# jcorsetti/oryon

Hardware: AMD Instinct MI355X
Metric: image-pairs/sec end-to-end (feat+match+reg) @224², C=256; ADD(-S) parity (higher is better)
Workload: dtype f32

## Files before the change

### oryon_amd/csrc/screen_mx6.hip

```cpp
#include <hip/hip_runtime.h>
#include <stdio.h>
#include <stdlib.h>
#include <type_traits>
#include "common.h"
#include "match_common.h"
#include "screen_tile.h"

namespace oryon {

typedef int i32x8 __attribute__((ext_vector_type(8)));
typedef float f32x16s __attribute__((ext_vector_type(16)));

template <int CP, int WAVES = 8, int VAR = 0>
__global__ __launch_bounds__(64 * WAVES, CP == 512 ? 1 : 2) void match_mx6_screen_kernel(
    const uint8_t *__restrict__ a6, const uint8_t *__restrict__ q6, int B, int cap_a, int cap_q, const int32_t *__restrict__ n_a,
    const int32_t *__restrict__ n_q, int T, int S, float *__restrict__ ws_max, int32_t *__restrict__ ws_i1, float *__restrict__ ws_m2)
{
    constexpr int RB = CP;
    constexpr int TILE_BYTES = screen8_tile_bytes(CP);
    constexpr int NQB = 4, NAB = 2;
    constexpr int NKS = CP / 64;
    constexpr int NI = TILE_BYTES / (1024 * WAVES);
    char *smem;
    if constexpr (2 * TILE_BYTES > 65536) {
        extern __shared__ __attribute__((aligned(256))) char smem_dyn6[];
        smem = smem_dyn6;
    } else {
        __shared__ __attribute__((aligned(256))) char smem_st6[2 * TILE_BYTES];
        smem = smem_st6;
    }
    ScreenUnit u;
    if (!screen_unit_decode(u, 64 * WAVES, B, T, S, n_a, n_q)) return;
    const int p = u.p, split = u.split, a0 = u.a0;
    int qt_begin, qt_end;
    screen_split_tiles(u, S, qt_begin, qt_end);
    const int t = threadIdx.x, lane = t & 63, wave = t >> 6, l31 = lane & 31, hi = lane >> 5;
    const char *qp = reinterpret_cast<const char *>(q6) + (size_t)p * cap_q * RB;

    i32x8 breg[NAB][NKS];
#pragma unroll
    for (int ab = 0; ab < NAB; ++ab) {
        const int arow_i = a0 + wave * 64 + ab * 32 + l31;
        const char *arow = reinterpret_cast<const char *>(a6) + ((size_t)p * cap_a + (arow_i < cap_a ? arow_i : cap_a - 1)) * RB + 32 * hi;
#pragma unroll
        for (int s = 0; s < NKS; ++s) {
            const i32x4 lo = *reinterpret_cast<const i32x4 *>(arow + 64 * s), up = *reinterpret_cast<const i32x4 *>(arow + 64 * s + 16);
            breg[ab][s] = __builtin_shufflevector(lo, up, 0, 1, 2, 3, 4, 5, 6, 7);
        }
    }
    unsigned dma_off[NI];
    screen_dma_offsets<RB>(dma_off, wave * NI, lane);
    const int wave_u = __builtin_amdgcn_readfirstlane(wave);
    auto issue_one = [&](int qt, int buf, int j) {
        const char *qb = qp + (size_t)qt * TILE_BYTES;
        char *dst = smem + buf * TILE_BYTES + (wave_u * NI + j) * 1024;
        __builtin_amdgcn_global_load_lds((const __attribute__((address_space(1))) void *)(qb + dma_off[j]),
                                         (__attribute__((address_space(3))) void *)dst, 16, 0, 0);
    };
    unsigned koff[4][2];
#pragma unroll
    for (int c = 0; c < 4; ++c)
#pragma unroll
        for (int e = 0; e < 2; ++e) koff[c][e] = (unsigned)(l31 * RB) + ((((unsigned)(4 * c + 2 * hi + e)) ^ (unsigned)(l31 & 15)) << 4);
    auto rd = [&](int s, int qb, unsigned tile) -> i32x8 {
        const unsigned base = tile + (unsigned)(qb * 32 * RB + (s >> 2) * 256);
        const i32x4 lo = *reinterpret_cast<const i32x4 *>(smem + koff[s & 3][0] + base);
        const i32x4 up = *reinterpret_cast<const i32x4 *>(smem + koff[s & 3][1] + base);
        return __builtin_shufflevector(lo, up, 0, 1, 2, 3, 4, 5, 6, 7);
    };

    float runmax[NAB], run2[NAB];
    int runidx[NAB];
#pragma unroll
    for (int ab = 0; ab < NAB; ++ab) { runmax[ab] = -INFINITY; run2[ab] = -INFINITY; runidx[ab] = 0; }
    auto reduce_block = [&](const f32x16s &c, int sid, int ab) {
        if constexpr (VAR == 1) { runmax[ab] = fmaxf(runmax[ab], c[0] + c[15]); runidx[ab] = sid; return; }
        const float m0 = fmaxf(fmaxf(c[0], c[1]), c[2]), m1 = fmaxf(fmaxf(c[3], c[4]), c[5]), m2 = fmaxf(fmaxf(c[6], c[7]), c[8]);
        const float m3 = fmaxf(fmaxf(c[9], c[10]), c[11]), m4 = fmaxf(fmaxf(c[12], c[13]), c[14]);
        const float x = fmaxf(fmaxf(fmaxf(m0, m1), m2), fmaxf(fmaxf(m3, m4), c[15]));
        const bool improved = x > runmax[ab];
        run2[ab] = __builtin_amdgcn_fmed3f(runmax[ab], run2[ab], x);
        runmax[ab] = fmaxf(runmax[ab], x);
        runidx[ab] = improved ? sid : runidx[ab];
    };
    const f32x16s zero16 = {0, 0, 0, 0, 0, 0, 0, 0, 0, 0, 0, 0, 0, 0, 0, 0};

    if (qt_end > qt_begin) {
#pragma unroll
        for (int j = 0; j < NI; ++j) issue_one(qt_begin, 0, j);
    }
    asm volatile("s_waitcnt vmcnt(0)" ::: "memory");
    __syncthreads();

    i32x8 areg[NKS];
#pragma unroll
    for (int s = 0; s < NKS; ++s) areg[s] = rd(s, 0, 0u);
    f32x16s prev[NAB];
#pragma unroll
    for (int ab = 0; ab < NAB; ++ab)
#pragma unroll
        for (int r = 0; r < 16; ++r) prev[ab][r] = -3.0e38f;
    int prev_sid = 0;
    auto do_tile = [&](int qt, auto BUFC) {
        constexpr int BUF = decltype(BUFC)::value;
        constexpr unsigned tile = BUF * TILE_BYTES;
        const int qt_next = qt + 1 < qt_end ? qt + 1 : qt;
#pragma unroll
        for (int qb = 0; qb < NQB; ++qb) {
            f32x16s acc[NAB];
            if (qb == 0) {
#pragma unroll
                for (int j = 0; j < NI; ++j) issue_one(qt_next, BUF ^ 1, j);
            }
#pragma unroll
            for (int s = 0; s < NKS; ++s) {
#pragma unroll
                for (int ab = 0; ab < NAB; ++ab)
                    acc[ab] = __builtin_amdgcn_mfma_scale_f32_32x32x64_f8f6f4(areg[s], breg[ab][s], s == 0 ? zero16 : acc[ab], 2, 2, 0,
                                                                               areg[s][6], 0, breg[ab][s][6]);
                if (qb + 1 < NQB) areg[s] = rd(s, qb + 1, tile);
            }
#pragma unroll
            for (int ab = 0; ab < NAB; ++ab) reduce_block(prev[ab], prev_sid, ab);
#pragma unroll
            for (int i = 0; i < NKS; ++i) {
                __builtin_amdgcn_sched_group_barrier(0x008, 1, 0);
                __builtin_amdgcn_sched_group_barrier(0x002, 24 / (2 * NKS), 0);
                __builtin_amdgcn_sched_group_barrier(0x008, 1, 0);
                __builtin_amdgcn_sched_group_barrier(0x002, 24 / (2 * NKS), 0);
                if (qb + 1 < NQB) __builtin_amdgcn_sched_group_barrier(0x100, 2, 0);
            }
#pragma unroll
            for (int ab = 0; ab < NAB; ++ab) prev[ab] = acc[ab];
            prev_sid = (qt * NQB + qb) * 2 + hi;
        }
        asm volatile("s_waitcnt vmcnt(0)" ::: "memory");
        __syncthreads();
#pragma unroll
        for (int s = 0; s < NKS; ++s) areg[s] = rd(s, 0, (BUF ^ 1) * TILE_BYTES);
    };
    for (int qt = qt_begin; qt < qt_end; qt += 2) {
        do_tile(qt, std::integral_constant<int, 0>{});
        if (qt + 1 < qt_end) do_tile(qt + 1, std::integral_constant<int, 1>{});
    }
#pragma unroll
    for (int ab = 0; ab < NAB; ++ab) reduce_block(prev[ab], prev_sid, ab);
    screen_merge_store<NAB>(runmax, run2, runidx, a0 + wave * 64 + l31, hi, (size_t)p * S + split, cap_a, ws_max, ws_i1, ws_m2);
}


template <int S0, int N, class F>
__device__ __forceinline__ void mx6_static_for(F &&f)
{
    if constexpr (S0 < N) {
        f(std::integral_constant<int, S0>{});
        mx6_static_for<S0 + 1, N>(f);
    }
}

struct Mx6RowList {
    const int32_t *idx;
    int idx_stride, stride, cap_src;
    int n;
};
struct Mx6RowsInPlace {};

template <int CP, int WAVES, int KL, bool IDX = false>
__device__ __forceinline__ void mx6_screen_w4_tiles(char *smem, const uint8_t *__restrict__ a6, const uint8_t *__restrict__ q6, int p, int split,
                                                    int a0, int cap_a, int cap_q, int S, int qt_begin, int qt_end, float *__restrict__ ws_max,
                                                    int32_t *__restrict__ ws_i1, float *__restrict__ ws_m2,
                                                    const std::conditional_t<IDX, Mx6RowList, Mx6RowsInPlace> &rows = {})
{
    static_assert(CP == 256 || (CP == 512 && WAVES == 4), "geometries: C_pad 256 with 4 / 8 waves, C_pad 512 with 4 waves");
    constexpr int RB = CP, NAB = 4;
    constexpr int TILE_BYTES = screen8_tile_bytes(CP);
    constexpr int NQB = 4;
    constexpr int NKS = CP / 64;
    constexpr int NI = TILE_BYTES / (1024 * WAVES);
    constexpr int LPR = RB / 256;
    const int t = threadIdx.x, lane = t & 63, wave = t >> 6, l31 = lane & 31, hi = lane >> 5;
    const char *qp = reinterpret_cast<const char *>(q6) + (size_t)p * cap_q * RB;

    i32x8 breg[NAB][NKS];
    int bsc[NAB][NKS / 4];
#pragma unroll
    for (int ab = 0; ab < NAB; ++ab) {
        const int arow_i = a0 + wave * (32 * NAB) + ab * 32 + l31;
        const char *arow;
        bool live = true;
        if constexpr (IDX) {
            live = arow_i < rows.n;
            const int src = !live ? 0 : rows.idx ? rows.idx[(size_t)p * rows.idx_stride + arow_i] : arow_i * rows.stride;
            arow = reinterpret_cast<const char *>(a6) + ((size_t)p * rows.cap_src + src) * RB + 32 * hi;
        } else
            arow = reinterpret_cast<const char *>(a6) + ((size_t)p * cap_a + (arow_i < cap_a ? arow_i : cap_a - 1)) * RB + 32 * hi;
        unsigned sc[NKS / 4];
#pragma unroll
        for (int w = 0; w < NKS / 4; ++w) sc[w] = 0;
#pragma unroll
        for (int s = 0; s < KL; ++s) {
            i32x4 lo = *reinterpret_cast<const i32x4 *>(arow + 64 * s), up = *reinterpret_cast<const i32x4 *>(arow + 64 * s + 16);
            if constexpr (IDX) {
                const i32x4 z = {0, 0, 0, 0};
                lo = live ? lo : z;
                up = live ? up : z;
            }
            breg[ab][s] = __builtin_shufflevector(lo, up, 0, 1, 2, 3, 4, 5, -1, -1);
            sc[s >> 2] |= ((unsigned)up[2] & 0xffu) << (8 * (s & 3));
        }
#pragma unroll
        for (int w = 0; w < NKS / 4; ++w) bsc[ab][w] = (int)sc[w];
    }
    constexpr int DJ = 4 * LPR;
    static_assert(NI % DJ == 0 || NI == DJ, "DMA instructions per wave and tile");
    unsigned dma_off[DJ];
    screen_dma_offsets<RB>(dma_off, wave * NI, lane);
    const int wave_u = __builtin_amdgcn_readfirstlane(wave);
    auto issue_one = [&](int qt, int buf, int j) {
        const char *qb = qp + (size_t)qt * TILE_BYTES + (j / DJ) * (16 * RB);
        char *dst = smem + buf * TILE_BYTES + (wave_u * NI + j) * 1024;
        __builtin_amdgcn_global_load_lds((const __attribute__((address_space(1))) void *)(qb + dma_off[j % DJ]),
                                         (__attribute__((address_space(3))) void *)dst, 16, 0, 0);
    };
    unsigned koff[4][2];
#pragma unroll
    for (int c = 0; c < 4; ++c)
#pragma unroll
        for (int e = 0; e < 2; ++e) koff[c][e] = (unsigned)(l31 * RB) + ((((unsigned)(4 * c + 2 * hi + e)) ^ (unsigned)(l31 & 15)) << 4);
    auto rd = [&](int s, int qb, unsigned tile) -> i32x8 {
        const unsigned base = tile + (unsigned)(qb * 32 * RB + (s >> 2) * 256);
        const i32x4 lo = *reinterpret_cast<const i32x4 *>(smem + koff[s & 3][0] + base);
        const i32x4 up = *reinterpret_cast<const i32x4 *>(smem + koff[s & 3][1] + base);
        return __builtin_shufflevector(lo, up, 0, 1, 2, 3, 4, 5, 6, -1);
    };

    float runmax[NAB], run2[NAB];
    int runidx[NAB];
#pragma unroll
    for (int ab = 0; ab < NAB; ++ab) { runmax[ab] = -INFINITY; run2[ab] = -INFINITY; runidx[ab] = 0; }
    auto reduce_block = [&](const f32x16s &c, int sid, int ab) {
        const float m0 = fmaxf(fmaxf(c[0], c[1]), c[2]), m1 = fmaxf(fmaxf(c[3], c[4]), c[5]), m2 = fmaxf(fmaxf(c[6], c[7]), c[8]);
        const float m3 = fmaxf(fmaxf(c[9], c[10]), c[11]), m4 = fmaxf(fmaxf(c[12], c[13]), c[14]);
        const float x = fmaxf(fmaxf(fmaxf(m0, m1), m2), fmaxf(fmaxf(m3, m4), c[15]));
        const bool improved = x > runmax[ab];
        run2[ab] = __builtin_amdgcn_fmed3f(runmax[ab], run2[ab], x);
        runmax[ab] = __builtin_amdgcn_fmed3f(runmax[ab], x, INFINITY);
        runidx[ab] = improved ? sid : runidx[ab];
    };
    const f32x16s zero16 = {0, 0, 0, 0, 0, 0, 0, 0, 0, 0, 0, 0, 0, 0, 0, 0};

    if (qt_end > qt_begin) {
#pragma unroll
        for (int j = 0; j < NI; ++j) issue_one(qt_begin, 0, j);
    }
    asm volatile("s_waitcnt vmcnt(0)" ::: "memory");
    __syncthreads();

    i32x8 areg[NKS];
#pragma unroll
    for (int s = 0; s < KL; ++s) areg[s] = rd(s, 0, 0u);
    f32x16s acc[NAB];
#pragma unroll
    for (int ab = 0; ab < NAB; ++ab)
#pragma unroll
        for (int r = 0; r < 16; ++r) acc[ab][r] = -3.0e38f;
    int sid23 = 0;

    auto mfma = [&](f32x16s &d, int ab, auto SC) {
        constexpr int s_ = decltype(SC)::value;
        d = __builtin_amdgcn_mfma_scale_f32_32x32x64_f8f6f4(areg[s_], breg[ab][s_], s_ == 0 ? zero16 : d, 2, 2, 0, areg[s_][6], s_ & 3,
                                                            bsc[ab][s_ >> 2]);
    };
    int buf = 0;
    for (int qt = qt_begin; qt < qt_end; ++qt) {
        const unsigned tile = buf * TILE_BYTES;
        const int qt_next = qt + 1 < qt_end ? qt + 1 : qt;
#pragma unroll
        for (int qb = 0; qb < NQB; ++qb) {
            const int sid = (qt * NQB + qb) * 2 + hi;
            if (qb == 0) {
#pragma unroll
                for (int j = 0; j < NI; ++j) issue_one(qt_next, buf ^ 1, j);
            }
            reduce_block(acc[2], sid23, 2);
            reduce_block(acc[3], sid23, 3);
            mx6_static_for<0, KL>([&](auto SC) { mfma(acc[0], 0, SC); mfma(acc[1], 1, SC); });
#pragma unroll
            for (int i = 0; i < 2 * KL; ++i) {
                __builtin_amdgcn_sched_group_barrier(0x008, 1, 0);
                __builtin_amdgcn_sched_group_barrier(0x002, 16 / KL, 0);
            }
            mx6_static_for<0, KL>([&](auto SC) {
                constexpr int s_ = decltype(SC)::value;
                mfma(acc[2], 2, SC); mfma(acc[3], 3, SC);
                if (qb + 1 < NQB) areg[s_] = rd(s_, qb + 1, tile);
            });
            reduce_block(acc[0], sid, 0);
            reduce_block(acc[1], sid, 1);
#pragma unroll
            for (int i = 0; i < 2 * KL; ++i) {
                __builtin_amdgcn_sched_group_barrier(0x008, 1, 0);
                __builtin_amdgcn_sched_group_barrier(0x002, 16 / KL, 0);
                if (qb + 1 < NQB && (i & 1)) __builtin_amdgcn_sched_group_barrier(0x100, 2, 0);
            }
            sid23 = sid;
        }
        asm volatile("s_waitcnt vmcnt(0)" ::: "memory");
        __syncthreads();
        buf ^= 1;
#pragma unroll
        for (int s = 0; s < KL; ++s) areg[s] = rd(s, 0, buf * TILE_BYTES);
    }
    reduce_block(acc[2], sid23, 2);
    reduce_block(acc[3], sid23, 3);
    screen_merge_store<NAB>(runmax, run2, runidx, a0 + wave * (32 * NAB) + l31, hi, (size_t)p * S + split, cap_a, ws_max, ws_i1, ws_m2);
}

template <int CP, int WAVES, int KL = CP / 64>
__global__ __launch_bounds__(64 * WAVES, CP == 512 ? 1 : 2) void match_mx6_screen_w4_kernel(
    const uint8_t *__restrict__ a6, const uint8_t *__restrict__ q6, int B, int cap_a, int cap_q, const int32_t *__restrict__ n_a,
    const int32_t *__restrict__ n_q, int T, int S, float *__restrict__ ws_max, int32_t *__restrict__ ws_i1, float *__restrict__ ws_m2,
    long long *__restrict__ dbg_wg )
{
    constexpr int TILE_BYTES = screen8_tile_bytes(CP);
    char *smem;
    if constexpr (2 * TILE_BYTES > 65536) {
        extern __shared__ __attribute__((aligned(256))) char smem_dyn_w4[];
        smem = smem_dyn_w4;
    } else {
        __shared__ __attribute__((aligned(256))) char smem_st_w4[2 * TILE_BYTES];
        smem = smem_st_w4;
    }
    ScreenUnit u;
    if (!screen_unit_decode(u, 128 * WAVES, B, T, S, n_a, n_q)) return;
    int qt_begin, qt_end;
    screen_split_tiles(u, S, qt_begin, qt_end);
    const long long tk0 = dbg_wg ? wall_clock64() : 0;
    mx6_screen_w4_tiles<CP, WAVES, KL>(smem, a6, q6, u.p, u.split, u.a0, cap_a, cap_q, S, qt_begin, qt_end, ws_max, ws_i1, ws_m2);
    if (dbg_wg && threadIdx.x == 0) {
        dbg_wg[(size_t)blockIdx.x * 4 + 0] = tk0;
        dbg_wg[(size_t)blockIdx.x * 4 + 1] = wall_clock64();
        dbg_wg[(size_t)blockIdx.x * 4 + 2] = (long long)__builtin_amdgcn_s_getreg((31 << 11) | 4);
        dbg_wg[(size_t)blockIdx.x * 4 + 3] = (long long)__builtin_amdgcn_s_getreg((31 << 11) | 20);
    }
}

template <int KL>
__global__ __launch_bounds__(256, 2) void match_mx6_screen_w4_list_kernel(
    const uint8_t *__restrict__ a6, const uint8_t *__restrict__ q6, int B, int cap_src, int cap_list, int cap_q, const int32_t *__restrict__ count,
    const int32_t *__restrict__ idx, int idx_stride, int stride, const int32_t *__restrict__ n_q, int T, int S, float *__restrict__ ws_max,
    int32_t *__restrict__ ws_i1, float *__restrict__ ws_m2)
{
    __shared__ __attribute__((aligned(256))) char smem_st_w4l[2 * screen8_tile_bytes(256)];
    ScreenUnit u;
    if (!screen_unit_decode(u, 512, B, T, S, count, n_q)) return;
    Mx6RowList rows = {idx, idx_stride, stride, cap_src, 0};
    const int listed = idx ? u.na : (u.na + stride - 1) / stride;
    rows.n = listed < cap_list ? listed : cap_list;
    if (u.a0 >= rows.n) return;
    int qt_begin, qt_end;
    screen_split_tiles(u, S, qt_begin, qt_end);
    mx6_screen_w4_tiles<256, 4, KL, true>(smem_st_w4l, a6, q6, u.p, u.split, u.a0, cap_list, cap_q, S, qt_begin, qt_end, ws_max, ws_i1, ws_m2, rows);
}

template <int CP, int WAVES, int KL = CP / 64>
__global__ __launch_bounds__(64 * WAVES, CP == 512 ? 1 : 2) void match_mx6_screen_w4_win_kernel(
    const uint8_t *__restrict__ a6, const uint8_t *__restrict__ q6, int B, int cap_a, int cap_q, const int32_t *__restrict__ n_a,
    const int32_t *__restrict__ n_q, int T, int S, float *__restrict__ ws_max, int32_t *__restrict__ ws_i1, float *__restrict__ ws_m2,
    const int32_t *__restrict__ gate , int win ,
    const int32_t *__restrict__ band ,
    int band_T )
{
    constexpr int TILE_BYTES = screen8_tile_bytes(CP);
    char *smem;
    if constexpr (2 * TILE_BYTES > 65536) {
        extern __shared__ __attribute__((aligned(256))) char smem_dyn_w4w[];
        smem = smem_dyn_w4w;
    } else {
        __shared__ __attribute__((aligned(256))) char smem_st_w4w[2 * TILE_BYTES];
        smem = smem_st_w4w;
    }
    ScreenUnit u;
    if (!screen_unit_decode(u, 128 * WAVES, B, T, S, n_a, n_q)) return;
    if (gate && gate[u.p * T + u.panel] == 0) return;
    int qt_begin, qt_end;
    screen_split_tiles(u, S, qt_begin, qt_end);
    if (win > 0 && qt_end - qt_begin > win) {
        const int cnt = qt_end - qt_begin, panels = (u.na + 128 * WAVES - 1) / (128 * WAVES);
        int k0 = (int)(((long long)(2 * u.panel + 1) * cnt) / (2 * panels)) - win / 2;
        k0 = k0 < 0 ? 0 : (k0 > cnt - win ? cnt - win : k0);
        qt_begin += k0;
        qt_end = qt_begin + win;
    }
    if (band) {
        const int first = band[(u.p * band_T + u.panel) * 2], cnt = band[(u.p * band_T + u.panel) * 2 + 1];
        const int per = (cnt + S - 1) / S;
        qt_begin = first + u.split * per;
        qt_end = (qt_begin + per < first + cnt) ? qt_begin + per : first + cnt;
    }
    mx6_screen_w4_tiles<CP, WAVES, KL>(smem, a6, q6, u.p, u.split, u.a0, cap_a, cap_q, S, qt_begin, qt_end, ws_max, ws_i1, ws_m2);
}

static int mx6_var()
{
    static const int var = dev_env_int("ORYON_MX6_VAR", 0);
    return var;
}

namespace {
int mx6_live_ksteps(int C_true) { return (C_true > 0 && C_true <= 64) ? 1 : (C_true > 0 && C_true <= 128) ? 2 : 4; }
template <class F>
void mx6_with_kl(int kl, F &&f)
{
    if (kl == 1) f(std::integral_constant<int, 1>{});
    else if (kl == 2) f(std::integral_constant<int, 2>{});
    else f(std::integral_constant<int, 4>{});
}

template <int CP>
void launch_screen_mx6_t(int groups, int T, hipStream_t st, const uint8_t *a6, const uint8_t *q6, int B, int cap_a, int cap_q, const int32_t *n_a,
                       const int32_t *n_q, int S, float *ws_max, int32_t *ws_i1, float *ws_m2, int kl = 4, bool gate_or_win = false,
                       const int32_t *gate = nullptr, int win = 0)
{
    constexpr size_t dyn = 2 * screen8_tile_bytes(CP) > 65536 ? 2 * screen8_tile_bytes(CP) : 0;
    constexpr int W_ = CP == 512 ? 4 : 8;
    const int Tw = (cap_a + 64 * W_ - 1) / (64 * W_);
    const int var = mx6_var();
    if (var == 1) {
        if (dyn) allow_dynamic_lds(reinterpret_cast<const void *>(&match_mx6_screen_kernel<CP, W_, 1>), (int)dyn);
        hipLaunchKernelGGL((match_mx6_screen_kernel<CP, W_, 1>), dim3(groups / T * Tw), dim3(64 * W_), dyn, st, a6, q6, B, cap_a, cap_q, n_a, n_q, Tw,
                           S, ws_max, ws_i1, ws_m2);
        return;
    }
    if constexpr (CP == 256) {
        if (var == 0) {
            const int T8 = (cap_a + 1023) / 1024;
            const int g8 = groups / T * T8;
            if (gate_or_win) {
                mx6_with_kl(kl, [&](auto KLC) {
                    hipLaunchKernelGGL((match_mx6_screen_w4_win_kernel<CP, 8, decltype(KLC)::value>), dim3(g8), dim3(512), 0, st, a6, q6, B, cap_a,
                                       cap_q, n_a, n_q, T8, S, ws_max, ws_i1, ws_m2, gate, win, static_cast<const int32_t *>(nullptr), 0);
                });
                return;
            }
            mx6_with_kl(kl, [&](auto KLC) {
                hipLaunchKernelGGL((match_mx6_screen_w4_kernel<CP, 8, decltype(KLC)::value>), dim3(g8), dim3(512), 0, st, a6, q6, B, cap_a, cap_q,
                                   n_a, n_q, T8, S, ws_max, ws_i1, ws_m2, static_cast<long long *>(nullptr));
            });
            return;
        }
        if (var == 3) {
            hipLaunchKernelGGL((match_mx6_screen_w4_kernel<CP, 4>), dim3(groups / T * Tw), dim3(256), 0, st, a6, q6, B, cap_a, cap_q, n_a, n_q, Tw, S,
                               ws_max, ws_i1, ws_m2, nullptr);
            return;
        }
    }
    if constexpr (CP == 512) {
        if (var == 0) {
            allow_dynamic_lds(reinterpret_cast<const void *>(&match_mx6_screen_w4_kernel<CP, 4>), (int)dyn);
            hipLaunchKernelGGL((match_mx6_screen_w4_kernel<CP, 4>), dim3(groups / T * Tw), dim3(256), dyn, st, a6, q6, B, cap_a, cap_q, n_a, n_q, Tw,
                               S, ws_max, ws_i1, ws_m2, nullptr);
            return;
        }
    }
    if (dyn) allow_dynamic_lds(reinterpret_cast<const void *>(&match_mx6_screen_kernel<CP, W_>), (int)dyn);
    hipLaunchKernelGGL((match_mx6_screen_kernel<CP, W_>), dim3(groups / T * Tw), dim3(64 * W_), dyn, st, a6, q6, B, cap_a, cap_q, n_a, n_q, Tw, S,
                       ws_max, ws_i1, ws_m2);
}
}

const char *screen_mx6_name(int C)
{
    if (C != 256) return mx6_var() == 0 ? "match_mx6_screen_w4_kernel<512, 4>" : "match_mx6_screen_kernel<512, 4, 0>";
    return mx6_var() == 0 ? "match_mx6_screen_w4_kernel<256, 8>" : mx6_var() == 3 ? "match_mx6_screen_w4_kernel<256, 4>" : mx6_var() == 1 ? "match_mx6_screen_kernel<256, 8, 1>" : "match_mx6_screen_kernel<256, 8, 0>";
}

void launch_screen_mx6(int C, int groups, int T, hipStream_t st, const uint8_t *a6, const uint8_t *q6, int B, int cap_a, int cap_q,
                       const int32_t *n_a, const int32_t *n_q, int S, float *ws_max, int32_t *ws_i1, float *ws_m2, int C_true,
                       int cascade, const int32_t *gate, int win)
{
    if (C == 256)
        launch_screen_mx6_t<256>(groups, T, st, a6, q6, B, cap_a, cap_q, n_a, n_q, S, ws_max, ws_i1, ws_m2, mx6_live_ksteps(C_true), cascade != 0,
                                 gate, win);
    else launch_screen_mx6_t<512>(groups, T, st, a6, q6, B, cap_a, cap_q, n_a, n_q, S, ws_max, ws_i1, ws_m2);
}

void launch_screen_mx6_list512(hipStream_t st, const uint8_t *a6, const uint8_t *q6, int B, int cap_src, int cap_list, int cap_q,
                               const int32_t *count, const int32_t *idx, int idx_stride, int stride, const int32_t *n_q, int S, float *ws_max,
                               int32_t *ws_i1, float *ws_m2, int C_true)
{
    const int T = (cap_list + 511) / 512;
    const int groups = ((B * S + 7) / 8) * 8 * T;
    mx6_with_kl(mx6_live_ksteps(C_true), [&](auto KLC) {
        hipLaunchKernelGGL((match_mx6_screen_w4_list_kernel<decltype(KLC)::value>), dim3(groups), dim3(256), 0, st, a6, q6, B, cap_src, cap_list,
                           cap_q, count, idx, idx_stride, stride, n_q, T, S, ws_max, ws_i1, ws_m2);
    });
}

void launch_screen_mx6_band512(hipStream_t st, const uint8_t *a6, const uint8_t *q6, int B, int cap_a, int cap_q, const int32_t *n_a,
                               const int32_t *n_q, int S, float *ws_max, int32_t *ws_i1, float *ws_m2, int C_true, const int32_t *band, int band_T)
{
    const int T = (cap_a + 511) / 512;
    const int groups = ((B * S + 7) / 8) * 8 * T;
    mx6_with_kl(mx6_live_ksteps(C_true), [&](auto KLC) {
        hipLaunchKernelGGL((match_mx6_screen_w4_win_kernel<256, 4, decltype(KLC)::value>), dim3(groups), dim3(256), 0, st, a6, q6, B, cap_a, cap_q,
                           n_a, n_q, T, S, ws_max, ws_i1, ws_m2, static_cast<const int32_t *>(nullptr), 0, band, band_T);
    });
}

}
```

### oryon_amd/csrc/screen_tile.h

```cpp
#pragma once
#include <hip/hip_runtime.h>
#include <stdint.h>

namespace oryon {

typedef int i32x4 __attribute__((ext_vector_type(4)));

constexpr int SCREEN8_ROWS = 128;
constexpr int screen8_tile_bytes(int CP) { return CP * SCREEN8_ROWS; }

struct ScreenUnit {
    int p, split, panel, a0, na, nq;
};
__device__ __forceinline__ bool screen_unit_decode(ScreenUnit &u, int panel_rows, int B, int T, int S, const int32_t *__restrict__ n_a,
                                                   const int32_t *__restrict__ n_q)
{
    const int xcd = blockIdx.x & 7, slot = blockIdx.x >> 3;
    const int unit = (slot / T) * 8 + xcd;
    if (unit >= B * S) return false;
    u.panel = slot % T;
    u.p = unit / S;
    u.split = unit % S;
    u.na = n_a[u.p];
    u.nq = n_q[u.p];
    u.a0 = u.panel * panel_rows;
    return u.a0 < u.na;
}
__device__ __forceinline__ void screen_split_tiles(const ScreenUnit &u, int S, int &qt_begin, int &qt_end)
{
    const int nqt = (u.nq + SCREEN8_ROWS - 1) / SCREEN8_ROWS;
    const int qt_per = (nqt + S - 1) / S;
    qt_begin = u.split * qt_per;
    qt_end = (qt_begin + qt_per < nqt) ? qt_begin + qt_per : nqt;
}

template <int RB, int N>
__device__ __forceinline__ void screen_dma_offsets(unsigned (&off)[N], int first, int lane)
{
    constexpr int LPR = RB / 256;
    static_assert(LPR >= 1, "rows are whole 256-byte lines");
#pragma unroll
    for (int j = 0; j < N; ++j) {
        const int line = (first + j) * 4 + (lane >> 4), sl = lane & 15;
        const int row = line / LPR;
        off[j] = (unsigned)(row * RB + (((line % LPR) * 16 + (sl ^ (row & 15))) << 4));
    }
}

template <int NAB>
__device__ __forceinline__ void screen_merge_store(const float (&runmax)[NAB], const float (&run2)[NAB], const int (&runidx)[NAB], int a_lane,
                                                   int hi, size_t unit, int cap_a, float *__restrict__ ws_max, int32_t *__restrict__ ws_i1,
                                                   float *__restrict__ ws_m2)
{
#pragma unroll
    for (int ab = 0; ab < NAB; ++ab) {
        const float om1 = __shfl_xor(runmax[ab], 32), om2 = __shfl_xor(run2[ab], 32);
        const int oi1 = __shfl_xor(runidx[ab], 32);
        const float m1 = fmaxf(runmax[ab], om1);
        const float m2 = fmaxf(fminf(runmax[ab], om1), fmaxf(run2[ab], om2));
        const int i1 = (om1 > runmax[ab]) ? oi1 : runidx[ab];
        const int a = a_lane + ab * 32;
        if (hi == 0 && a < cap_a) {
            const size_t o = unit * cap_a + a;
            ws_max[o] = m1;
            ws_i1[o] = i1;
            ws_m2[o] = m2;
        }
    }
}

}
```

Baseline: 23710.

## Skip dead A-row blocks on partial list panels in mx6 screen kernel

For list-indexed screening panels, rows are re-laid out so each 128-row level spans all waves, and the kernel is instantiated with 2, 3 or 4 live A blocks based on how many rows remain in the panel. Tail panels then issue fewer MFMAs and reductions instead of computing on zero-padded rows. The sched_group_barrier interleave is generalized to uneven halves. This adds extra template instantiations, which cost code size, and gives tail panels a different instruction schedule.

```diff
diff --git a/oryon_amd/csrc/screen_mx6.hip b/oryon_amd/csrc/screen_mx6.hip
--- a/oryon_amd/csrc/screen_mx6.hip
+++ b/oryon_amd/csrc/screen_mx6.hip
@@ -165,7 +165,7 @@
 };
 struct Mx6RowsInPlace {};
 
-template <int CP, int WAVES, int KL, bool IDX = false>
+template <int CP, int WAVES, int KL, bool IDX = false, int NABL = 4>
 __device__ __forceinline__ void mx6_screen_w4_tiles(char *smem, const uint8_t *__restrict__ a6, const uint8_t *__restrict__ q6, int p, int split,
                                                     int a0, int cap_a, int cap_q, int S, int qt_begin, int qt_end, float *__restrict__ ws_max,
                                                     int32_t *__restrict__ ws_i1, float *__restrict__ ws_m2,
@@ -173,6 +173,9 @@
 {
     static_assert(CP == 256 || (CP == 512 && WAVES == 4), "geometries: C_pad 256 with 4 / 8 waves, C_pad 512 with 4 waves");
     constexpr int RB = CP, NAB = 4;
+    static_assert(NABL == NAB || (IDX && NABL >= 2 && NABL < NAB), "live levels: 2 .. 4, fewer than 4 on list panels only");
+    constexpr int HA = (NABL + 1) / 2, HB = NABL - HA;
+    static_assert((16 * HB) % (HA * KL) == 0 && (16 * HA) % (HB * KL) == 0, "epilogue instructions per MFMA (sched_group_barrier)");
     constexpr int TILE_BYTES = screen8_tile_bytes(CP);
     constexpr int NQB = 4;
     constexpr int NKS = CP / 64;
@@ -184,8 +187,8 @@
     i32x8 breg[NAB][NKS];
     int bsc[NAB][NKS / 4];
 #pragma unroll
-    for (int ab = 0; ab < NAB; ++ab) {
-        const int arow_i = a0 + wave * (32 * NAB) + ab * 32 + l31;
+    for (int ab = 0; ab < NABL; ++ab) {
+        const int arow_i = IDX ? a0 + (ab * WAVES + wave) * 32 + l31 : a0 + wave * (32 * NAB) + ab * 32 + l31;
         const char *arow;
         bool live = true;
         if constexpr (IDX) {
@@ -261,7 +264,7 @@
     for (int s = 0; s < KL; ++s) areg[s] = rd(s, 0, 0u);
     f32x16s acc[NAB];
 #pragma unroll
-    for (int ab = 0; ab < NAB; ++ab)
+    for (int ab = 0; ab < NABL; ++ab)
 #pragma unroll
         for (int r = 0; r < 16; ++r) acc[ab][r] = -3.0e38f;
     int sid23 = 0;
@@ -282,26 +285,30 @@
 #pragma unroll
                 for (int j = 0; j < NI; ++j) issue_one(qt_next, buf ^ 1, j);
             }
-            reduce_block(acc[2], sid23, 2);
-            reduce_block(acc[3], sid23, 3);
-            mx6_static_for<0, KL>([&](auto SC) { mfma(acc[0], 0, SC); mfma(acc[1], 1, SC); });
-#pragma unroll
-            for (int i = 0; i < 2 * KL; ++i) {
+            if constexpr (HB > 0) reduce_block(acc[HA], sid23, HA);
+            if constexpr (HB > 1) reduce_block(acc[HA + 1], sid23, HA + 1);
+            mx6_static_for<0, KL>([&](auto SC) {
+                mfma(acc[0], 0, SC);
+                if constexpr (HA > 1) mfma(acc[1], 1, SC);
+            });
+#pragma unroll
+            for (int i = 0; i < HA * KL; ++i) {
                 __builtin_amdgcn_sched_group_barrier(0x008, 1, 0);
-                __builtin_amdgcn_sched_group_barrier(0x002, 16 / KL, 0);
+                __builtin_amdgcn_sched_group_barrier(0x002, 16 * HB / (HA * KL), 0);
             }
             mx6_static_for<0, KL>([&](auto SC) {
                 constexpr int s_ = decltype(SC)::value;
-                mfma(acc[2], 2, SC); mfma(acc[3], 3, SC);
+                if constexpr (HB > 0) mfma(acc[HA], HA, SC);
+                if constexpr (HB > 1) mfma(acc[HA + 1], HA + 1, SC);
                 if (qb + 1 < NQB) areg[s_] = rd(s_, qb + 1, tile);
             });
             reduce_block(acc[0], sid, 0);
-            reduce_block(acc[1], sid, 1);
-#pragma unroll
-            for (int i = 0; i < 2 * KL; ++i) {
+            if constexpr (HA > 1) reduce_block(acc[1], sid, 1);
+#pragma unroll
+            for (int i = 0; i < HB * KL; ++i) {
                 __builtin_amdgcn_sched_group_barrier(0x008, 1, 0);
-                __builtin_amdgcn_sched_group_barrier(0x002, 16 / KL, 0);
-                if (qb + 1 < NQB && (i & 1)) __builtin_amdgcn_sched_group_barrier(0x100, 2, 0);
+                __builtin_amdgcn_sched_group_barrier(0x002, 16 * HA / (HB * KL), 0);
+                if (qb + 1 < NQB && i % HB == HB - 1) __builtin_amdgcn_sched_group_barrier(0x100, 2, 0);
             }
             sid23 = sid;
         }
@@ -311,9 +318,10 @@
 #pragma unroll
         for (int s = 0; s < KL; ++s) areg[s] = rd(s, 0, buf * TILE_BYTES);
     }
-    reduce_block(acc[2], sid23, 2);
-    reduce_block(acc[3], sid23, 3);
-    screen_merge_store<NAB>(runmax, run2, runidx, a0 + wave * (32 * NAB) + l31, hi, (size_t)p * S + split, cap_a, ws_max, ws_i1, ws_m2);
+    if constexpr (HB > 0) reduce_block(acc[HA], sid23, HA);
+    if constexpr (HB > 1) reduce_block(acc[HA + 1], sid23, HA + 1);
+    screen_merge_store<NAB, NABL>(runmax, run2, runidx, a0 + (IDX ? wave * 32 : wave * (32 * NAB)) + l31, hi, (size_t)p * S + split, cap_a, ws_max,
+                                  ws_i1, ws_m2, IDX ? 32 * WAVES : 32);
 }
 
 template <int CP, int WAVES, int KL = CP / 64>
@@ -360,7 +368,16 @@
     if (u.a0 >= rows.n) return;
     int qt_begin, qt_end;
     screen_split_tiles(u, S, qt_begin, qt_end);
-    mx6_screen_w4_tiles<256, 4, KL, true>(smem_st_w4l, a6, q6, u.p, u.split, u.a0, cap_list, cap_q, S, qt_begin, qt_end, ws_max, ws_i1, ws_m2, rows);
+    const int levels = (rows.n - u.a0 + 127) >> 7;
+    if (levels >= 4) {
+        mx6_screen_w4_tiles<256, 4, KL, true, 4>(smem_st_w4l, a6, q6, u.p, u.split, u.a0, cap_list, cap_q, S, qt_begin, qt_end, ws_max, ws_i1, ws_m2, rows);
+        return;
+    }
+    if (levels == 3) {
+        mx6_screen_w4_tiles<256, 4, KL, true, 3>(smem_st_w4l, a6, q6, u.p, u.split, u.a0, cap_list, cap_q, S, qt_begin, qt_end, ws_max, ws_i1, ws_m2, rows);
+        return;
+    }
+    mx6_screen_w4_tiles<256, 4, KL, true, 2>(smem_st_w4l, a6, q6, u.p, u.split, u.a0, cap_list, cap_q, S, qt_begin, qt_end, ws_max, ws_i1, ws_m2, rows);
 }
 
 template <int CP, int WAVES, int KL = CP / 64>
diff --git a/oryon_amd/csrc/screen_tile.h b/oryon_amd/csrc/screen_tile.h
--- a/oryon_amd/csrc/screen_tile.h
+++ b/oryon_amd/csrc/screen_tile.h
@@ -47,19 +47,20 @@
     }
 }
 
-template <int NAB>
+template <int NAB, int NLIVE = NAB>
 __device__ __forceinline__ void screen_merge_store(const float (&runmax)[NAB], const float (&run2)[NAB], const int (&runidx)[NAB], int a_lane,
                                                    int hi, size_t unit, int cap_a, float *__restrict__ ws_max, int32_t *__restrict__ ws_i1,
-                                                   float *__restrict__ ws_m2)
+                                                   float *__restrict__ ws_m2, int ab_stride = 32)
 {
+    static_assert(NLIVE >= 1 && NLIVE <= NAB, "live blocks of a lane");
 #pragma unroll
-    for (int ab = 0; ab < NAB; ++ab) {
+    for (int ab = 0; ab < NLIVE; ++ab) {
         const float om1 = __shfl_xor(runmax[ab], 32), om2 = __shfl_xor(run2[ab], 32);
         const int oi1 = __shfl_xor(runidx[ab], 32);
         const float m1 = fmaxf(runmax[ab], om1);
         const float m2 = fmaxf(fminf(runmax[ab], om1), fmaxf(run2[ab], om2));
         const int i1 = (om1 > runmax[ab]) ? oi1 : runidx[ab];
-        const int a = a_lane + ab * 32;
+        const int a = a_lane + ab * ab_stride;
         if (hi == 0 && a < cap_a) {
             const size_t o = unit * cap_a + a;
             ws_max[o] = m1;
```

Result: no change. 23860 (median of 6 runs) (+0.6%).
